# fugue-project/fugue

Measured on NVIDIA H100. Metric: transform() rows/sec, hash-partitioned (num=256) identity map, 8-col table, higher is better.
Workload: dtype int64+f64 (byte moves; u64 hash arithmetic)

## Files before the change

### fugue_b200/csrc/fb_partition.cu

```cuda
#include <stdlib.h>

#include <mutex>

#include "fb_common.cuh"

namespace {

constexpr int kBlock = 512;
constexpr int kItems = 8;
constexpr int kTile = kBlock * kItems;
constexpr int kWarps = kBlock / 32;
constexpr int kCtasPerSm = 2;

struct FbCols {
  const void* src[FB_MAX_COLS];
  void* dst[FB_MAX_COLS];
  int32_t width[FB_MAX_COLS];
  int32_t ncols;
};

struct ChunkGeom {
  int64_t nrows;
  int64_t full_rows;
  int64_t tiles_per_chunk;
// ... 278 lines not shown
  uint64_t* buf;
  uint32_t* delta;
  uint32_t* cursor;
  uint32_t* bin_start;
  uint32_t* cnt;
  uint32_t* scanw;
  uint16_t* pid_sorted;
  uint32_t nbp;
};

template <typename T, bool kFull>
__device__ __forceinline__ void load_col(const void* __restrict__ src, int64_t warp_row0, int warp_rows,
                                         unsigned lane, T (&v)[kItems]) {
  const T* __restrict__ p = (const T*)src + warp_row0 + lane;
#pragma unroll
  for (int r = 0; r < kItems; ++r)
    if (kFull || r * 32 + (int)lane < warp_rows) v[r] = __ldg(p + r * 32);
}

template <typename T, bool kFull>
__device__ __forceinline__ void move_columns(const FbCols& cols, const TileCtx& cx,
                                             const uint32_t (&pos)[kItems], const uint32_t (&dst)[kItems],
                                             int64_t warp_row0, int warp_rows, int tile_rows,
                                             unsigned lane, int& phase) {
  int c = 0;
  while (c < cols.ncols && cols.width[c] != (int)sizeof(T)) ++c;
  if (c >= cols.ncols) return;
  T v[kItems];
  load_col<T, kFull>(cols.src[c], warp_row0, warp_rows, lane, v);
  while (c < cols.ncols) {
    T* __restrict__ buf = (T*)(cx.buf + (size_t)(phase & 1) * kTile);
#pragma unroll
    for (int r = 0; r < kItems; ++r) buf[pos[r]] = v[r];
    int nxt = c + 1;
    while (nxt < cols.ncols && cols.width[nxt] != (int)sizeof(T)) ++nxt;
    if (nxt < cols.ncols) load_col<T, kFull>(cols.src[nxt], warp_row0, warp_rows, lane, v);
    __syncthreads();
    T* __restrict__ out = (T*)cols.dst[c];
#pragma unroll
    for (int k = 0; k < kItems; ++k) {
      const int j = k * kBlock + (int)threadIdx.x;
      if (kFull || j < tile_rows) out[dst[k]] = buf[j];
    }
    ++phase;
    c = nxt;
  }
}

template <bool kSingleU64, int kBits, bool kFull, bool kAll8>
__device__ __forceinline__ void scatter_tile(const FbKeys& keys, const FbDiv& dv, const uint32_t num,
                                             const FbCols& cols, const TileCtx& cx,
                                             const int64_t tile_row0, const int tile_rows, int& phase) {
  const unsigned lane = threadIdx.x & 31, warp = threadIdx.x >> 5;
  const unsigned lt = fb_lanemask_lt();
  const uint32_t nb = num + 1;
  const uint32_t nbp = cx.nbp;
  uint32_t* __restrict__ my_cnt = cx.cnt + warp * nbp;
  const int64_t warp_row0 = tile_row0 + (int64_t)warp * (32 * kItems);
  const int warp_rows = tile_rows - (int)warp * (32 * kItems);

  uint32_t pid[kItems];
#pragma unroll
  for (int r = 0; r < kItems; ++r) {
    const bool ok = kFull || (r * 32 + (int)lane) < warp_rows;
    pid[r] = ok ? compute_pid<kSingleU64>(keys, dv, warp_row0 + r * 32 + lane) : num;
  }

  uint32_t pos[kItems];
#pragma unroll
  for (int r = 0; r < kItems; ++r) {
    const unsigned m = match_lanes<kBits + (kFull ? 0 : 1)>(pid[r], 0xFFFFFFFFu);
    const unsigned before = __popc(m & lt);
    uint32_t old = 0;
    if (before == 0) {
      old = my_cnt[pid[r]];
      my_cnt[pid[r]] = old + __popc(m);
    }
    __syncwarp();
    old = __shfl_sync(0xFFFFFFFFu, old, __ffs(m) - 1);
    pos[r] = old + before;
  }
  __syncthreads();

  {
    const uint32_t per = (nb + kBlock - 1) / kBlock;
    const uint32_t b0 = threadIdx.x * per;
    uint32_t tot[kMaxPer];
    uint32_t sum = 0;
#pragma unroll
    for (int i = 0; i < kMaxPer; ++i) {
      tot[i] = 0;
      if ((uint32_t)i < per && b0 + i < nb) {
        uint32_t run = 0;
#pragma unroll
        for (int w = 0; w < kWarps; ++w) {
          const uint32_t t = cx.cnt[w * nbp + b0 + i];
          cx.cnt[w * nbp + b0 + i] = run;
          run += t;
        }
        tot[i] = run;
        sum += run;
      }
    }
    uint32_t x = sum;
#pragma unroll
    for (int o = 1; o < 32; o <<= 1) {
      const uint32_t y = __shfl_up_sync(0xFFFFFFFFu, x, o);
      if (lane >= (unsigned)o) x += y;
    }
    if (lane == 31) cx.scanw[warp] = x;
    __syncthreads();
    uint32_t run = x - sum;
    {
      const uint32_t wt = lane < kWarps ? cx.scanw[lane] : 0;
#pragma unroll
      for (int w = 0; w < kWarps; ++w) {
        const uint32_t v = __shfl_sync(0xFFFFFFFFu, wt, w);
        if ((unsigned)w < warp) run += v;
      }
    }
#pragma unroll
    for (int i = 0; i < kMaxPer; ++i) {
      if ((uint32_t)i < per && b0 + i < nb) {
        const uint32_t cur = cx.cursor[b0 + i];
        cx.bin_start[b0 + i] = run;
        cx.delta[b0 + i] = cur - run;
        cx.cursor[b0 + i] = cur + tot[i];
        run += tot[i];
      }
    }
  }
  __syncthreads();

#pragma unroll
  for (int r = 0; r < kItems; ++r) {
    pos[r] += cx.bin_start[pid[r]] + my_cnt[pid[r]];
    cx.pid_sorted[pos[r]] = (uint16_t)pid[r];
  }
  __syncthreads();
  uint32_t dst[kItems];
#pragma unroll
  for (int k = 0; k < kItems; ++k) {
    const int j = k * kBlock + (int)threadIdx.x;
    dst[k] = cx.delta[cx.pid_sorted[j]] + (uint32_t)j;
  }
  for (uint32_t i = threadIdx.x; i < (uint32_t)kWarps * nbp; i += kBlock) cx.cnt[i] = 0;

  move_columns<uint64_t, kFull>(cols, cx, pos, dst, warp_row0, warp_rows, tile_rows, lane, phase);
  if (!kAll8) {
    move_columns<uint32_t, kFull>(cols, cx, pos, dst, warp_row0, warp_rows, tile_rows, lane, phase);
    move_columns<uint16_t, kFull>(cols, cx, pos, dst, warp_row0, warp_rows, tile_rows, lane, phase);
    move_columns<uint8_t, kFull>(cols, cx, pos, dst, warp_row0, warp_rows, tile_rows, lane, phase);
  }
  __syncthreads();
}

template <bool kSingleU64, int kBits, bool kAll8>
__global__ void __launch_bounds__(kBlock, kCtasPerSm)
fb_scatter_kernel(FbKeys keys, FbDiv dv, uint32_t num, ChunkGeom g, int chunk0,
                  const uint32_t* __restrict__ chunk_base, const int64_t* __restrict__ part_offsets,
                  FbCols cols) {
  extern __shared__ __align__(128) uint64_t smem64[];
  TileCtx cx;
  cx.nbp = nb_padded(num);
  cx.buf = smem64;
  cx.delta = (uint32_t*)(smem64 + 2 * kTile);
  cx.cursor = cx.delta + cx.nbp;
  cx.bin_start = cx.cursor + cx.nbp;
  cx.cnt = cx.bin_start + cx.nbp;
  cx.scanw = cx.cnt + kWarps * cx.nbp;
  cx.pid_sorted = (uint16_t*)(cx.scanw + 32);

  const int chunk = chunk0 + (int)blockIdx.x;
  int64_t chunk_row0, chunk_row1;
  chunk_range(g, chunk, chunk_row0, chunk_row1);

  for (uint32_t b = threadIdx.x; b < cx.nbp; b += kBlock)
    cx.cursor[b] = b < num ? (uint32_t)part_offsets[b] + chunk_base[(size_t)chunk * num + b] : 0u;
  for (uint32_t i = threadIdx.x; i < (uint32_t)kWarps * cx.nbp; i += kBlock) cx.cnt[i] = 0;
  __syncthreads();

  int phase = 0;
  for (int64_t tile_row0 = chunk_row0; tile_row0 < chunk_row1; tile_row0 += kTile) {
    const int64_t left = chunk_row1 - tile_row0;
    if (left >= kTile)
      scatter_tile<kSingleU64, kBits, true, kAll8>(keys, dv, num, cols, cx, tile_row0, kTile, phase);
    else
      scatter_tile<kSingleU64, kBits, false, kAll8>(keys, dv, num, cols, cx, tile_row0, (int)left, phase);
  }
}

constexpr int kSwcMaxCols = 8;
constexpr uint32_t kSwcMaxNum = 256;

__device__ __forceinline__ uint32_t smem_u32(const void* p) { return (uint32_t)__cvta_generic_to_shared(p); }

__device__ __forceinline__ void mbar_init(uint32_t bar, uint32_t count) {
  asm volatile("mbarrier.init.shared::cta.b64 [%0], %1;" ::"r"(bar), "r"(count) : "memory");
}
__device__ __forceinline__ void mbar_expect_tx(uint32_t bar, uint32_t bytes) {
  asm volatile("mbarrier.arrive.expect_tx.shared::cta.b64 _, [%0], %1;" ::"r"(bar), "r"(bytes) : "memory");
}
__device__ __forceinline__ void mbar_arrive_relaxed(uint32_t bar) {
  asm volatile("mbarrier.arrive.relaxed.cta.shared::cta.b64 _, [%0];" ::"r"(bar) : "memory");
}
__device__ __forceinline__ void mbar_wait(uint32_t bar, uint32_t parity) {
  asm volatile(
      "{\n"
      ".reg .pred p;\n"
      "FB_WAIT:\n"
      "mbarrier.try_wait.parity.shared::cta.b64 p, [%0], %1;\n"
      "@p bra FB_DONE;\n"
      "bra FB_WAIT;\n"
      "FB_DONE:\n"
      "}\n" ::"r"(bar), "r"(parity)
      : "memory");
}
__device__ __forceinline__ uint64_t l2_policy_evict_first() {
  uint64_t pol;
  asm volatile("createpolicy.fractional.L2::evict_first.b64 %0, 1.0;" : "=l"(pol));
  return pol;
}
__device__ __forceinline__ uint64_t l2_policy_evict_last() {
  uint64_t pol;
  asm volatile("createpolicy.fractional.L2::evict_last.b64 %0, 1.0;" : "=l"(pol));
  return pol;
}
__device__ __forceinline__ void tma_load_1d(uint32_t dst_smem, const void* src, uint32_t bytes, uint32_t bar,
                                            uint64_t policy) {
  asm volatile(
      "cp.async.bulk.shared::cluster.global.mbarrier::complete_tx::bytes.L2::cache_hint [%0], [%1], %2, [%3], %4;"
      ::"r"(dst_smem), "l"(src), "r"(bytes), "r"(bar), "l"(policy)
      : "memory");
}

constexpr int kWsMoverWarps = 16, kWsRankWarps = 8;
constexpr int kWsMovers = kWsMoverWarps * 32, kWsRankers = kWsRankWarps * 32;
constexpr int kWsThreads = kWsMovers + kWsRankers + 128;
constexpr int kWsG = 4;
constexpr int kWsRankItems = 16;

struct WsUnits {
  const uint64_t* src[FB_MAX_COLS];
  uint64_t* dst[FB_MAX_COLS];
  int32_t nunits;
  int32_t per_group;
  int32_t ngroups;
};

struct WsMap {
  const uint64_t* src2[FB_MAX_COLS];
  uint64_t a[FB_MAX_COLS], b[FB_MAX_COLS], c[FB_MAX_COLS];
  int32_t mode[FB_MAX_COLS];
};

__device__ __forceinline__ uint64_t ws_apply_map(int mode, bool two, uint64_t x, uint64_t y, uint64_t a, uint64_t b,
                                                 uint64_t c) {
  if (mode == 1) {
    double r = __dmul_rn(__longlong_as_double((long long)a), __longlong_as_double((long long)x));
    if (two) r = __dadd_rn(r, __dmul_rn(__longlong_as_double((long long)b), __longlong_as_double((long long)y)));
    return (uint64_t)__double_as_longlong(__dadd_rn(r, __longlong_as_double((long long)c)));
  }
  if (mode == 2) return a * x + (two ? b * y : 0ULL) + c;
  return x;
}

template <int G, int RI>
__host__ __device__ inline size_t ws_book_bytes(uint32_t num, int ncols) {
  constexpr size_t kT = (size_t)kWsRankers * RI;
  const size_t nbp = nb_padded(num);
  const size_t E = (size_t)num * (G - 1);
  size_t b = 64 * 8;
  b += (size_t)ncols * E * 8;
  b += (kT + E) * 4;
  b += 6 * nbp * 4 + 64 * 4;
  b += ((E * 2 + 15) / 16) * 16;
  b += 2 * (size_t)kMetaBytes + 128;
  return b;
}

__device__ __forceinline__ void mbar_arrive(uint32_t bar) {
  asm volatile("mbarrier.arrive.shared::cta.b64 _, [%0];" ::"r"(bar) : "memory");
}
__device__ __forceinline__ void mover_sync() { asm volatile("bar.sync 1, %0;" ::"n"(kWsMovers) : "memory"); }
__device__ __forceinline__ void ranker_sync() { asm volatile("bar.sync 2, %0;" ::"n"(kWsRankers) : "memory"); }

template <int kBits, int G, int kWsRankItems, bool kMap>
__global__ void __launch_bounds__(kWsThreads, 1)
fb_scatter_ws_kernel(WsUnits units, uint32_t num, ChunkGeom g, int nstages,
                     const uint8_t* __restrict__ meta,
                     const uint32_t* __restrict__ chunk_base, const int64_t* __restrict__ part_offsets,
                     const __grid_constant__ WsMap map) {
  constexpr uint32_t T = (uint32_t)kWsRankers * kWsRankItems;
  static_assert(T == (uint32_t)kTile, "pass 1 ranks tiles of kTile rows");
  constexpr uint32_t GM = G - 1;
  constexpr uint32_t kStageBytes = T * 8;
  constexpr int kSlotRounds = ((int)T + (int)kSwcMaxNum * (G - 1) + kWsMovers - 1) / kWsMovers;
  constexpr int kEntryRoundsM = ((int)kSwcMaxNum * (G - 1) + kWsMovers - 1) / kWsMovers;
  constexpr int kEntryRoundsR = ((int)kSwcMaxNum * (G - 1) + kWsRankers - 1) / kWsRankers;
  extern __shared__ __align__(128) uint64_t smem64[];
  const uint32_t nbp = nb_padded(num);
  const uint32_t E = num * GM;
  const int grp = (int)blockIdx.x % units.ngroups;
  const int chunk_first = (int)blockIdx.x / units.ngroups, chunk_step = (int)gridDim.x / units.ngroups;
  const int u0 = grp * units.per_group;
  const int ncols = min(units.per_group, units.nunits - u0);
  uint64_t* ring = smem64;
  uint64_t* bars = ring + (size_t)nstages * T;
  uint64_t* carry = bars + 64;
  uint32_t* slotinfo = (uint32_t*)(carry + (size_t)ncols * E);
  uint32_t* wpos = slotinfo + T + E;
  uint32_t* kcnt = wpos + nbp;
  uint32_t* binfo = kcnt + nbp;
  uint32_t* bin_n = binfo + nbp;
  uint32_t* wstart = bin_n + nbp;
  uint32_t* wdelta = wstart + nbp;
  uint32_t* scanw = wdelta + nbp;
  uint16_t* carryinfo = (uint16_t*)(scanw + 64);
  uint8_t* metabuf = (uint8_t*)(((uintptr_t)(carryinfo + E) + 127) & ~(uintptr_t)127);

  const unsigned lane = threadIdx.x & 31, warp = threadIdx.x >> 5;
  const uint32_t bar_full = smem_u32(bars), bar_empty = smem_u32(bars + 16);
  const uint32_t bar_pid_full = smem_u32(bars + 32), bar_pid_empty = smem_u32(bars + 34);
  const uint32_t bar_slots_ready = smem_u32(bars + 36), bar_slots_free = smem_u32(bars + 37);
  const uint32_t bar_flush_done = smem_u32(bars + 38);
  const uint32_t bar_carry_read = smem_u32(bars + 40);

  if (threadIdx.x == 0) {
    for (int s = 0; s < nstages; ++s) {
      mbar_init(bar_full + 8 * s, 1);
      mbar_init(bar_empty + 8 * s, kWsMoverWarps);
    }
    for (int i = 0; i < 2; ++i) {
      mbar_init(bar_pid_full + 8 * i, 1);
      mbar_init(bar_pid_empty + 8 * i, kWsRankWarps);
    }
    mbar_init(bar_slots_ready, kWsRankWarps);
    mbar_init(bar_slots_free, kWsMoverWarps);
    mbar_init(bar_flush_done, kWsMoverWarps);
    mbar_init(bar_carry_read, kWsMoverWarps);
    mbar_init(bar_carry_read + 8, kWsMoverWarps);
    asm volatile("fence.mbarrier_init.release.cluster;" ::: "memory");
  }
  __syncthreads();

  if (warp >= kWsMoverWarps + kWsRankWarps) {
    if (warp == kWsMoverWarps + kWsRankWarps && lane == 0) {
      const uint64_t pol = l2_policy_evict_first(), meta_pol = l2_policy_evict_last();
      const uint32_t ring_s = smem_u32(ring), meta_s = smem_u32(metabuf);
      uint32_t s = 0, ph = 0, seq = 0;
      int chunk = chunk_first;
      int64_t r0 = 0, r1 = 0, t0 = 0;
      bool have = chunk < g.nchunks_full;
      if (have) { chunk_range(g, chunk, r0, r1); t0 = r0; }
      auto load_pid = [&](int64_t row0, uint32_t q) {
        const uint32_t b = q & 1, pp = (q >> 1) & 1;
        mbar_wait(bar_pid_empty + 8 * b, pp ^ 1);
        mbar_expect_tx(bar_pid_full + 8 * b, kMetaBytes);
        tma_load_1d(meta_s + b * kMetaBytes, meta + (size_t)(row0 / T) * kMetaBytes, kMetaBytes,
                    bar_pid_full + 8 * b, meta_pol);
      };
      if (have) load_pid(t0, 0);
      while (have) {
        int nchunk = chunk;
        int64_t nr0 = r0, nr1 = r1, nt0 = t0 + T;
        bool nhave = true;
        if (nt0 >= r1) {
          nchunk = chunk + chunk_step;
          nhave = nchunk < g.nchunks_full;
          if (nhave) { chunk_range(g, nchunk, nr0, nr1); nt0 = nr0; }
        }
        if (nhave) load_pid(nt0, seq + 1);
        for (int u = u0; u < u0 + ncols; ++u) {
          mbar_wait(bar_empty + 8 * s, ph ^ 1);
          mbar_expect_tx(bar_full + 8 * s, kStageBytes);
          tma_load_1d(ring_s + s * kStageBytes, units.src[u] + t0, kStageBytes, bar_full + 8 * s, pol);
          if (++s == (uint32_t)nstages) { s = 0; ph ^= 1; }
          if constexpr (kMap) {
            if (map.src2[u] != nullptr) {
              mbar_wait(bar_empty + 8 * s, ph ^ 1);
              mbar_expect_tx(bar_full + 8 * s, kStageBytes);
              tma_load_1d(ring_s + s * kStageBytes, map.src2[u] + t0, kStageBytes, bar_full + 8 * s, pol);
              if (++s == (uint32_t)nstages) { s = 0; ph ^= 1; }
            }
          }
        }
        chunk = nchunk; r0 = nr0; r1 = nr1; t0 = nt0; have = nhave;
        ++seq;
      }
    }
    return;
  }

  if (warp >= kWsMoverWarps) {
    const unsigned rw = warp - kWsMoverWarps;
    const unsigned rtid = threadIdx.x - kWsMovers;
    uint32_t seq = 0, cseq = 0;
    for (int chunk = chunk_first; chunk < g.nchunks_full; chunk += chunk_step, ++cseq) {
      int64_t r0, r1;
      chunk_range(g, chunk, r0, r1);
      if (cseq > 0) mbar_wait(bar_flush_done, (cseq - 1) & 1);
      ranker_sync();
      for (uint32_t b = rtid; b < nbp; b += kWsRankers) {
        const uint32_t p0 = b < num ? (uint32_t)part_offsets[b] + chunk_base[(size_t)chunk * num + b] : 0u;
        wpos[b] = p0 & ~GM;
        kcnt[b] = (p0 & GM) | ((p0 & GM) << 8);
      }
      ranker_sync();
      for (int64_t t0 = r0; t0 < r1; t0 += T, ++seq) {
        const uint32_t pb = seq & 1, pph = (seq >> 1) & 1;
        mbar_wait(bar_pid_full + 8 * pb, pph);
        const uint8_t* __restrict__ rec = metabuf + pb * kMetaBytes;
        uint32_t pr[kWsRankItems];
#pragma unroll
        for (int r = 0; r < kWsRankItems; ++r) {
          const uint32_t row = r * kWsRankers + rtid;
          pr[r] = ((uint32_t)rec[row] << 16) | ((const uint16_t*)(rec + kMetaRank))[row];
        }
        const uint32_t b = rtid;
        uint32_t n = 0, w = 0, kold = 0, phold = 0, wp_old = 0;
        if (b < num) n = ((const uint16_t*)(rec + kMetaCnt))[b];
        __syncwarp();
        if (lane == 0) mbar_arrive_relaxed(bar_pid_empty + 8 * pb);
        if (b < num) {
          const uint32_t kc = kcnt[b];
          kold = kc & 0xFFu;
          phold = kc >> 8;
          wp_old = wpos[b];
          const uint32_t end = wp_old + kold + n;
          const uint32_t aend = end & ~GM;
          if (aend > wp_old) {
            w = aend - wp_old;
            wpos[b] = aend;
            kcnt[b] = end - aend;
          } else {
            kcnt[b] = (kold + n) | (phold << 8);
          }
          binfo[b] = kold | (phold << 4) | (w << 8);
          bin_n[b] = n;
        }
        uint32_t xw = w;
#pragma unroll
        for (int o = 1; o < 32; o <<= 1) {
          const uint32_t yw = __shfl_up_sync(0xFFFFFFFFu, xw, o);
          if (lane >= (unsigned)o) xw += yw;
        }
        if (lane == 31) scanw[8 + rw] = xw;
        ranker_sync();
        uint32_t bw = xw - w;
        {
          const uint32_t tw = lane < kWsRankWarps ? scanw[8 + lane] : 0;
#pragma unroll
          for (int wi = 0; wi < kWsRankWarps; ++wi) {
            const uint32_t vw = __shfl_sync(0xFFFFFFFFu, tw, wi);
            if ((unsigned)wi < rw) bw += vw;
          }
        }
        if (seq > 0) mbar_wait(bar_slots_free, (seq - 1) & 1);
        if (b < num) {
          wstart[b] = bw;
          wdelta[b] = wp_old - bw;
        }
        if (rtid == kWsRankers - 1) scanw[40] = bw + w;
        ranker_sync();
#pragma unroll
        for (int r = 0; r < kWsRankItems; ++r) {
          const uint32_t pb2 = pr[r] >> 16;
          const uint32_t bi = binfo[pb2];
          const uint32_t i = (bi & 0xFu) + (pr[r] & 0xFFFFu);
          const uint32_t ww = bi >> 8;
          const uint32_t row = r * kWsRankers + rtid;
          if (i < ww) slotinfo[wstart[pb2] + i] = (pb2 << 16) | row;
          else carryinfo[pb2 * GM + (i - ww)] = (uint16_t)row;
        }
#pragma unroll
        for (int q = 0; q < kEntryRoundsR; ++q) {
          const uint32_t e = q * kWsRankers + rtid;
          if (e < E) {
            const uint32_t eb = e / GM, i = e - eb * GM;
            const uint32_t bi = binfo[eb];
            const uint32_t ko = bi & 0xFu, po = (bi >> 4) & 0xFu, ww = bi >> 8;
            const uint32_t nn = bin_n[eb];
            const uint32_t desc = i < po ? 0xFFFFu : T + e;
            if (i < ko) {
              if (i < ww) slotinfo[wstart[eb] + i] = (eb << 16) | desc;
              else carryinfo[e] = (uint16_t)desc;
            }
            if (ww + i >= ko + nn) carryinfo[e] = 0xFFFFu;
          }
        }
        ranker_sync();
        if (lane == 0) mbar_arrive(bar_slots_ready);
      }
    }
    return;
  }

  uint32_t s = 0, ph = 0, seq = 0, astep = 0, wstep = 0;
  for (int chunk = chunk_first; chunk < g.nchunks_full; chunk += chunk_step) {
    int64_t r0, r1;
    chunk_range(g, chunk, r0, r1);
    for (int64_t t0 = r0; t0 < r1; t0 += T, ++seq) {
      mbar_wait(bar_slots_ready, seq & 1);
      const uint32_t W = scanw[40];
      uint32_t srcd[kSlotRounds], dst[kSlotRounds];
#pragma unroll
      for (int k = 0; k < kSlotRounds; ++k) {
        const uint32_t j = k * kWsMovers + threadIdx.x;
        srcd[k] = 0xFFFFu;
        dst[k] = 0;
        if (j < W) {
          const uint32_t info = slotinfo[j];
          srcd[k] = info & 0xFFFFu;
          dst[k] = wdelta[info >> 16] + j;
        }
      }
      uint32_t csrc[kEntryRoundsM];
#pragma unroll
      for (int q = 0; q < kEntryRoundsM; ++q) {
        const uint32_t e = q * kWsMovers + threadIdx.x;
        csrc[q] = e < E ? (uint32_t)carryinfo[e] : 0xFFFFu;
      }
      __syncwarp();
      if (lane == 0) mbar_arrive(bar_slots_free);

      uint64_t cv_prev[kEntryRoundsM];
      for (int u = 0; u < ncols; ++u) {
        mbar_wait(bar_full + 8 * s, ph);
        const uint64_t* __restrict__ st = ring + (size_t)s * T;
        uint64_t* __restrict__ out = units.dst[u0 + u];
        const uint64_t* __restrict__ cbuf = carry + (size_t)u * E;
        uint64_t v[kSlotRounds], cv[kEntryRoundsM];
        uint32_t s2 = s;
        bool two = false;
        if constexpr (kMap) {
          const int mode = map.mode[u0 + u];
          two = map.src2[u0 + u] != nullptr;
          const uint64_t* __restrict__ st2 = st;
          if (two) {
            s2 = s + 1 == (uint32_t)nstages ? 0 : s + 1;
            mbar_wait(bar_full + 8 * s2, s2 == 0 ? ph ^ 1 : ph);
            st2 = ring + (size_t)s2 * T;
          }
          const uint64_t ma = map.a[u0 + u], mb = map.b[u0 + u], mc = map.c[u0 + u];
#pragma unroll
          for (int k = 0; k < kSlotRounds; ++k)
            if (srcd[k] != 0xFFFFu)
              v[k] = srcd[k] < T ? ws_apply_map(mode, two, st[srcd[k]], st2[srcd[k]], ma, mb, mc) : cbuf[srcd[k] - T];
#pragma unroll
          for (int q = 0; q < kEntryRoundsM; ++q)
            if (csrc[q] != 0xFFFFu)
              cv[q] = csrc[q] < T ? ws_apply_map(mode, two, st[csrc[q]], st2[csrc[q]], ma, mb, mc) : cbuf[csrc[q] - T];
        } else {
#pragma unroll
          for (int k = 0; k < kSlotRounds; ++k)
            if (srcd[k] != 0xFFFFu) v[k] = srcd[k] < T ? st[srcd[k]] : cbuf[srcd[k] - T];
#pragma unroll
          for (int q = 0; q < kEntryRoundsM; ++q)
            if (csrc[q] != 0xFFFFu) cv[q] = csrc[q] < T ? st[csrc[q]] : cbuf[csrc[q] - T];
        }
#pragma unroll
        for (int k = 0; k < kSlotRounds; ++k)
          if (srcd[k] != 0xFFFFu) out[dst[k]] = v[k];
        __syncwarp();
        if (lane == 0) {
          mbar_arrive_relaxed(bar_empty + 8 * s);
          if (kMap && two) mbar_arrive_relaxed(bar_empty + 8 * s2);
          mbar_arrive_relaxed(bar_carry_read + 8 * (astep & 1));
        }
        ++astep;
        if (++s == (uint32_t)nstages) { s = 0; ph ^= 1; }
        if (kMap && two) {
          if (++s == (uint32_t)nstages) { s = 0; ph ^= 1; }
        }
        if (u > 0) {
          mbar_wait(bar_carry_read + 8 * (wstep & 1), (wstep >> 1) & 1);
          ++wstep;
          uint64_t* __restrict__ pbuf = carry + (size_t)(u - 1) * E;
#pragma unroll
          for (int q = 0; q < kEntryRoundsM; ++q) {
            const uint32_t e = q * kWsMovers + threadIdx.x;
            if (csrc[q] != 0xFFFFu) pbuf[e] = cv_prev[q];
          }
        }
#pragma unroll
        for (int q = 0; q < kEntryRoundsM; ++q) cv_prev[q] = cv[q];
      }
      {
        mbar_wait(bar_carry_read + 8 * (wstep & 1), (wstep >> 1) & 1);
        ++wstep;
        uint64_t* __restrict__ pbuf = carry + (size_t)(ncols - 1) * E;
#pragma unroll
        for (int q = 0; q < kEntryRoundsM; ++q) {
          const uint32_t e = q * kWsMovers + threadIdx.x;
          if (csrc[q] != 0xFFFFu) pbuf[e] = cv_prev[q];
        }
      }
    }
    mover_sync();
    for (int u = 0; u < ncols; ++u) {
      uint64_t* __restrict__ out = units.dst[u0 + u];
      const uint64_t* __restrict__ cbuf = carry + (size_t)u * E;
#pragma unroll
      for (int q = 0; q < kEntryRoundsM; ++q) {
        const uint32_t e = q * kWsMovers + threadIdx.x;
        if (e < E) {
          const uint32_t b = e / GM, i = e - b * GM;
          const uint32_t kc = kcnt[b];
          if (i < (kc & 0xFFu) && i >= (kc >> 8)) out[wpos[b] + i] = cbuf[e];
        }
      }
    }
    __syncwarp();
    if (lane == 0) mbar_arrive(bar_flush_done);
  }
}

__global__ void fb_bits_to_bytes_kernel(const uint8_t* __restrict__ bits, int64_t bit_offset,
                                        int64_t nrows, uint8_t* __restrict__ out) {
  int64_t i = (int64_t)blockIdx.x * blockDim.x + threadIdx.x;
  int64_t stride = (int64_t)gridDim.x * blockDim.x;
  for (; i < nrows; i += stride) {
    int64_t j = i + bit_offset;
    out[i] = (bits[j >> 3] >> (j & 7)) & 1;
  }
}

__global__ void fb_bytes_to_bits_kernel(const uint8_t* __restrict__ bytes, int64_t nrows,
                                        uint8_t* __restrict__ out, unsigned long long* null_count) {
  int64_t nbytes = (nrows + 7) >> 3;
  int64_t i = (int64_t)blockIdx.x * blockDim.x + threadIdx.x;
  int64_t stride = (int64_t)gridDim.x * blockDim.x;
  unsigned long long nulls = 0;
  for (; i < nbytes; i += stride) {
    uint8_t v = 0;
#pragma unroll
    for (int k = 0; k < 8; ++k) {
      int64_t r = i * 8 + k;
      if (r < nrows) {
        if (bytes[r]) v |= (uint8_t)(1u << k);
        else ++nulls;
      }
    }
    out[i] = v;
  }
  if (null_count != nullptr && nulls) atomicAdd(null_count, nulls);
}

inline int bits_for(uint32_t num) { return num <= 16 ? 4 : (num <= 256 ? 8 : 10); }

#define FB_DISPATCH_SB(single, bits, LAUNCH)                 \
  do {                                                       \
    if (single) {                                            \
      if (bits == 4) LAUNCH(true, 4);                        \
      else if (bits == 8) LAUNCH(true, 8);                   \
      else LAUNCH(true, 10);                                 \
    } else {                                                 \
      if (bits == 4) LAUNCH(false, 4);                       \
      else if (bits == 8) LAUNCH(false, 8);                  \
      else LAUNCH(false, 10);                                \
    }                                                        \
  } while (0)

template <typename K>
cudaError_t optin(K kernel, size_t bytes) {
  return cudaFuncSetAttribute(kernel, cudaFuncAttributeMaxDynamicSharedMemorySize, (int)bytes);
}

cudaError_t ensure_smem_optin(int dev) {
  static std::mutex mu;
  static uint64_t done = 0;
  std::lock_guard<std::mutex> lock(mu);
  if (dev >= 0 && dev < 64 && (done >> dev) & 1) return cudaSuccess;
  const size_t sc = scatter_smem_bytes(FB_MAX_PARTITIONS);
  const size_t hs = (size_t)kHistWarps * FB_MAX_PARTITIONS * sizeof(uint32_t);
  cudaError_t e = cudaSuccess;
#define FB_OPTIN(S, B)                                                   \
  do {                                                                   \
    if (e == cudaSuccess) e = optin(fb_scatter_kernel<S, B, true>, sc);  \
    if (e == cudaSuccess) e = optin(fb_scatter_kernel<S, B, false>, sc); \
    if (e == cudaSuccess) e = optin(fb_hist_kernel<S, B>, hs);           \
  } while (0)
  {
    int smem_max = 0;
    if (e == cudaSuccess) e = cudaDeviceGetAttribute(&smem_max, cudaDevAttrMaxSharedMemoryPerBlockOptin, dev);
    if (e == cudaSuccess) e = optin(fb_scatter_ws_kernel<4, kWsG, kWsRankItems, false>, (size_t)smem_max);
    if (e == cudaSuccess) e = optin(fb_scatter_ws_kernel<8, kWsG, kWsRankItems, false>, (size_t)smem_max);
    if (e == cudaSuccess) e = optin(fb_scatter_ws_kernel<4, kWsG, kWsRankItems, true>, (size_t)smem_max);
    if (e == cudaSuccess) e = optin(fb_scatter_ws_kernel<8, kWsG, kWsRankItems, true>, (size_t)smem_max);
  }
  if (e == cudaSuccess) e = optin(fb_rank_kernel<true, 4, true>, kRankStageBytes);
  if (e == cudaSuccess) e = optin(fb_rank_kernel<true, 8, true>, kRankStageBytes);
  if (e == cudaSuccess) e = optin(fb_rank_kernel<false, 4, true>, kRankStageBytes);
  if (e == cudaSuccess) e = optin(fb_rank_kernel<false, 8, true>, kRankStageBytes);
  FB_OPTIN(true, 4); FB_OPTIN(true, 8); FB_OPTIN(true, 10);
  FB_OPTIN(false, 4); FB_OPTIN(false, 8); FB_OPTIN(false, 10);
#undef FB_OPTIN
  if (e == cudaSuccess && dev >= 0 && dev < 64) done |= (1ull << dev);
  return e;
}

bool single_u64_key(int nkeys, const int32_t* widths, const uint8_t* const* valid) {
  return nkeys == 1 && widths[0] == 8 && (valid == nullptr || valid[0] == nullptr);
}

int fill_keys(FbKeys& k, int nkeys, const void* const* ptrs, const int32_t* widths,
              const uint8_t* const* valid) {
  FB_CHECK(nkeys >= 1 && nkeys <= FB_MAX_KEYS, "nkeys=%d out of range [1,%d]", nkeys, FB_MAX_KEYS);
  memset(&k, 0, sizeof(k));
  k.nkeys = nkeys;
  k.digit_shift = -1;
  for (int i = 0; i < nkeys; ++i) {
    FB_CHECK(widths[i] == 1 || widths[i] == 2 || widths[i] == 4 || widths[i] == 8,
             "key %d has unsupported width %d", i, widths[i]);
    FB_CHECK(ptrs[i] != nullptr, "key %d pointer is NULL", i);
    k.ptr[i] = ptrs[i];
    k.width[i] = widths[i];
    k.valid[i] = valid ? valid[i] : nullptr;
  }
  return 0;
}

struct PlanLayout {
  size_t hist_bytes;
  size_t pid_offset;
  size_t total_bytes;
};

PlanLayout plan_layout(const ChunkGeom& g, uint32_t num) {
  PlanLayout l;
  l.hist_bytes = (((size_t)g.nchunks * num * sizeof(uint32_t)) + 255) & ~(size_t)255;
  l.pid_offset = l.hist_bytes + 256;
  l.total_bytes = l.pid_offset + (num <= kSwcMaxNum ? (size_t)(g.full_rows / kTile) * kMetaBytes : 0) + 256;
  return l;
}

}

extern "C" {

size_t fb_partition_scratch_bytes(int dev, int64_t nrows, uint32_t num_partitions) {
  if (nrows < 0 || num_partitions == 0) return 0;
  ChunkGeom g = make_geom(dev, nrows);
  return plan_layout(g, num_partitions).total_bytes;
}

int fb_partition_ids(int dev, void* stream, int64_t nrows, int nkeys, const void* const* key_ptrs,
                     const int32_t* key_widths, const uint8_t* const* key_valid,
                     uint32_t num_partitions, uint32_t* out_pids) {
  FB_CHECK(nrows >= 0, "nrows < 0");
  FB_CHECK(num_partitions >= 1, "num_partitions must be >= 1");
  if (nrows == 0) return 0;
  FbDeviceGuard guard(dev);
  FB_CHECK(guard.ok, "cannot select device %d", dev);
  FbKeys k;
  if (int rc = fill_keys(k, nkeys, key_ptrs, key_widths, key_valid)) return rc;
  FbDiv dv = fb_make_div(num_partitions);
  int64_t blocks = (nrows + 255) / 256;
  int64_t maxb = (int64_t)fb_sm_count(dev) * 16;
  if (blocks > maxb) blocks = maxb;
  cudaStream_t st = (cudaStream_t)stream;
  if (single_u64_key(nkeys, key_widths, key_valid))
    fb_pid_kernel<true><<<(unsigned)blocks, 256, 0, st>>>(k, dv, nrows, out_pids);
  else
    fb_pid_kernel<false><<<(unsigned)blocks, 256, 0, st>>>(k, dv, nrows, out_pids);
  FB_CUDA(cudaGetLastError());
  return 0;
}

int fb_row_hash64(int dev, void* stream, int64_t nrows, int nkeys, const void* const* key_ptrs,
                  const int32_t* key_widths, const uint8_t* const* key_valid, uint64_t* out_hash) {
  FB_CHECK(nrows >= 0, "nrows < 0");
  if (nrows == 0) return 0;
  FbDeviceGuard guard(dev);
  FB_CHECK(guard.ok, "cannot select device %d", dev);
  FbKeys k;
  if (int rc = fill_keys(k, nkeys, key_ptrs, key_widths, key_valid)) return rc;
  int64_t blocks = (nrows + 255) / 256;
  int64_t maxb = (int64_t)fb_sm_count(dev) * 16;
  if (blocks > maxb) blocks = maxb;
  fb_row_hash_kernel<<<(unsigned)blocks, 256, 0, (cudaStream_t)stream>>>(k, nrows, out_hash);
  FB_CUDA(cudaGetLastError());
  return 0;
}

static int plan_impl(int dev, void* stream, int64_t nrows, const FbKeys& k, bool single,
                     uint32_t num_partitions, void* scratch, size_t scratch_bytes,
                     int64_t* out_part_offsets) {
  FB_CHECK(nrows >= 0, "nrows < 0");
  FB_CHECK(nrows < ((int64_t)1 << 32), "nrows=%lld exceeds the 2^32-1 rows one call handles",
           (long long)nrows);
  FB_CHECK(num_partitions >= 1 && num_partitions <= FB_MAX_PARTITIONS,
           "num_partitions=%u out of range [1,%d]", num_partitions, FB_MAX_PARTITIONS);
  FB_CHECK(out_part_offsets != nullptr, "out_part_offsets is NULL");
  FbDeviceGuard guard(dev);
  FB_CHECK(guard.ok, "cannot select device %d", dev);
  cudaStream_t st = (cudaStream_t)stream;
  if (nrows == 0) {
    FB_CUDA(cudaMemsetAsync(out_part_offsets, 0, sizeof(int64_t) * ((size_t)num_partitions + 1), st));
    return 0;
  }
  ChunkGeom g = make_geom(dev, nrows);
  PlanLayout l = plan_layout(g, num_partitions);
  FB_CHECK(scratch != nullptr && scratch_bytes >= l.total_bytes,
           "scratch too small: need %zu bytes, got %zu", l.total_bytes, scratch_bytes);
  FbDiv dv = fb_make_div(num_partitions);
  uint32_t* hist = (uint32_t*)scratch;
  size_t smem = (size_t)kHistWarps * num_partitions * sizeof(uint32_t);
  FB_CUDA(ensure_smem_optin(dev));
  const int bits = bits_for(num_partitions);
  int hist_chunk0 = 0;
  if (num_partitions <= kSwcMaxNum && g.nchunks_full > 0) {
    uint8_t* meta = (uint8_t*)scratch + l.pid_offset;
#define FB_LAUNCH_RANK(S, B, STAGED)                                                                  \
  fb_rank_kernel<S, B, STAGED><<<g.nchunks_full, kRankBlock, STAGED ? kRankStageBytes : 0, st>>>( \
      k, dv, num_partitions, g, hist, meta)
    if (single) {
      if (bits == 4) FB_LAUNCH_RANK(true, 4, true);
      else FB_LAUNCH_RANK(true, 8, true);
    } else if (k.digit_shift >= 0) {
      if (bits == 4) FB_LAUNCH_RANK(false, 4, true);
      else FB_LAUNCH_RANK(false, 8, true);
    } else {
      if (bits == 4) FB_LAUNCH_RANK(false, 4, false);
      else FB_LAUNCH_RANK(false, 8, false);
    }
#undef FB_LAUNCH_RANK
    FB_CUDA(cudaGetLastError());
    hist_chunk0 = g.nchunks_full;
  }
  if (hist_chunk0 < g.nchunks) {
#define FB_LAUNCH_HIST(S, B)                                                                       \
  fb_hist_kernel<S, B><<<g.nchunks - hist_chunk0, kHistBlock, smem, st>>>(k, dv, num_partitions, g, \
                                                                          hist_chunk0, hist)
    FB_DISPATCH_SB(single, bits, FB_LAUNCH_HIST);
#undef FB_LAUNCH_HIST
    FB_CUDA(cudaGetLastError());
  }
  fb_scan_chunks_kernel<<<num_partitions, 256, 0, st>>>(hist, num_partitions, g.nchunks, out_part_offsets);
  FB_CUDA(cudaGetLastError());
  fb_scan_parts_kernel<<<1, 1024, 0, st>>>(out_part_offsets, num_partitions);
  FB_CUDA(cudaGetLastError());
  return 0;
}

int fb_partition_plan(int dev, void* stream, int64_t nrows, int nkeys, const void* const* key_ptrs,
                      const int32_t* key_widths, const uint8_t* const* key_valid,
                      uint32_t num_partitions, void* scratch, size_t scratch_bytes,
                      int64_t* out_part_offsets) {
  FbKeys k;
  if (nrows == 0) {
    memset(&k, 0, sizeof(k));
    k.nkeys = 1;
    k.digit_shift = -1;
    return plan_impl(dev, stream, 0, k, false, num_partitions, scratch, scratch_bytes, out_part_offsets);
  }
  if (int rc = fill_keys(k, nkeys, key_ptrs, key_widths, key_valid)) return rc;
  return plan_impl(dev, stream, nrows, k, single_u64_key(nkeys, key_widths, key_valid), num_partitions,
                   scratch, scratch_bytes, out_part_offsets);
}

__global__ void fb_map_tail_kernel(int ncols, const void* const* __restrict__ x_ptrs, const fb_map_unit* __restrict__ maps,
                                   int64_t row0, int64_t nrows, uint64_t* __restrict__ tmp) {
  const int64_t n = nrows - row0;
  for (int64_t i = (int64_t)blockIdx.x * blockDim.x + threadIdx.x; i < n * ncols; i += (int64_t)gridDim.x * blockDim.x) {
    const int c = (int)(i / n);
    const int64_t r = row0 + i % n;
    const fb_map_unit m = maps[c];
    const uint64_t x = ((const uint64_t*)x_ptrs[c])[r];
    const uint64_t y = m.src2 != nullptr ? ((const uint64_t*)m.src2)[r] : 0;
    tmp[(size_t)c * kTile + (size_t)(i % n)] = ws_apply_map(m.mode, m.src2 != nullptr, x, y, m.a, m.b, m.c);
  }
}

static int apply_impl(int dev, void* stream, int64_t nrows, const FbKeys& k, bool single,
                      uint32_t num_partitions, const void* scratch, size_t scratch_bytes,
                      const int64_t* part_offsets, int ncols, const void* const* col_ptrs,
                      const int32_t* col_widths, void* const* out_col_ptrs, int sm_reserve = 0,
                      const fb_map_unit* maps = nullptr, void* tail_tmp = nullptr, int cols_per_launch_req = 0) {
  FB_CHECK(nrows >= 0 && nrows < ((int64_t)1 << 32), "nrows out of range");
  FB_CHECK(num_partitions >= 1 && num_partitions <= FB_MAX_PARTITIONS,
           "num_partitions=%u out of range [1,%d]", num_partitions, FB_MAX_PARTITIONS);
  FB_CHECK(ncols >= 0, "ncols < 0");
  if (nrows == 0 || ncols == 0) return 0;
  FbDeviceGuard guard(dev);
  FB_CHECK(guard.ok, "cannot select device %d", dev);
  ChunkGeom g = make_geom(dev, nrows);
  PlanLayout l = plan_layout(g, num_partitions);
  FB_CHECK(scratch != nullptr && scratch_bytes >= l.total_bytes, "scratch too small");
  FbDiv dv = fb_make_div(num_partitions);
  cudaStream_t st = (cudaStream_t)stream;
  const size_t smem = scatter_smem_bytes(num_partitions);
  FB_CUDA(ensure_smem_optin(dev));
  const int bits = bits_for(num_partitions);

  for (int c = 0; c < ncols; ++c) {
    const int w = col_widths[c];
    FB_CHECK(w == 1 || w == 2 || w == 4 || w == 8, "column %d has unsupported width %d", c, w);
    FB_CHECK(col_ptrs[c] != nullptr && out_col_ptrs[c] != nullptr, "column %d pointer is NULL", c);
  }

  const void* const* gen_src = col_ptrs;
  auto launch_generic = [&](const int* idx, int n, int chunk0, int nch) -> int {
    for (int c0 = 0; c0 < n && nch > 0; c0 += FB_MAX_COLS) {
      FbCols cols;
      memset(&cols, 0, sizeof(cols));
      cols.ncols = n - c0 < FB_MAX_COLS ? n - c0 : FB_MAX_COLS;
      bool all8 = true;
      for (int c = 0; c < cols.ncols; ++c) {
        cols.src[c] = gen_src[idx[c0 + c]];
        cols.dst[c] = out_col_ptrs[idx[c0 + c]];
        cols.width[c] = col_widths[idx[c0 + c]];
        all8 = all8 && cols.width[c] == 8;
      }
#define FB_LAUNCH_SCATTER(S, B)                                                                        \
  do {                                                                                                 \
    if (all8)                                                                                          \
// ... 230 lines not shown
```

Measured before the change: 16.10 billion.

## Assign each CTA a contiguous run of chunks to drop per-chunk flush barriers

The warp-specialized scatter kernel now gives each CTA one contiguous range of tiles instead of striding over chunks. Ranker state is seeded once from the first chunk's base, and the producer, ranker and mover loops iterate over tiles directly. This removes the per-chunk carry flush and the flush_done barrier between chunks, so the pipeline no longer drains at chunk boundaries. It relies on consecutive chunks' write positions continuing seamlessly. It also shifts load balance to the per-run split, which may be uneven when chunks do not divide evenly across runs.

```diff
diff --git a/fugue_b200/csrc/fb_partition.cu b/fugue_b200/csrc/fb_partition.cu
--- a/fugue_b200/csrc/fb_partition.cu
+++ b/fugue_b200/csrc/fb_partition.cu
@@ -604,7 +604,12 @@
   const uint32_t nbp = nb_padded(num);
   const uint32_t E = num * GM;
   const int grp = (int)blockIdx.x % units.ngroups;
-  const int chunk_first = (int)blockIdx.x / units.ngroups, chunk_step = (int)gridDim.x / units.ngroups;
+  const uint32_t run = blockIdx.x / (uint32_t)units.ngroups, nruns = gridDim.x / (uint32_t)units.ngroups;
+  const uint32_t c_lo = run * (uint32_t)g.nchunks_full / nruns;
+  const uint32_t c_hi = (run + 1) * (uint32_t)g.nchunks_full / nruns;
+  const uint32_t tile_lo = c_lo * (uint32_t)g.tiles_per_chunk;
+  const uint32_t tile_hi = min(c_hi * (uint32_t)g.tiles_per_chunk, (uint32_t)(g.full_rows / kTile));
+  const uint32_t run_tiles = tile_hi - tile_lo;
   const int u0 = grp * units.per_group;
   const int ncols = min(units.per_group, units.nunits - u0);
   uint64_t* ring = smem64;
@@ -625,7 +630,6 @@
   const uint32_t bar_full = smem_u32(bars), bar_empty = smem_u32(bars + 16);
   const uint32_t bar_pid_full = smem_u32(bars + 32), bar_pid_empty = smem_u32(bars + 34);
   const uint32_t bar_slots_ready = smem_u32(bars + 36), bar_slots_free = smem_u32(bars + 37);
-  const uint32_t bar_flush_done = smem_u32(bars + 38);
   const uint32_t bar_carry_read = smem_u32(bars + 40);
 
   if (threadIdx.x == 0) {
@@ -639,7 +643,6 @@
     }
     mbar_init(bar_slots_ready, kWsRankWarps);
     mbar_init(bar_slots_free, kWsMoverWarps);
-    mbar_init(bar_flush_done, kWsMoverWarps);
     mbar_init(bar_carry_read, kWsMoverWarps);
     mbar_init(bar_carry_read + 8, kWsMoverWarps);
     asm volatile("fence.mbarrier_init.release.cluster;" ::: "memory");
@@ -651,28 +654,17 @@
       const uint64_t pol = l2_policy_evict_first(), meta_pol = l2_policy_evict_last();
       const uint32_t ring_s = smem_u32(ring), meta_s = smem_u32(metabuf);
       uint32_t s = 0, ph = 0, seq = 0;
-      int chunk = chunk_first;
-      int64_t r0 = 0, r1 = 0, t0 = 0;
-      bool have = chunk < g.nchunks_full;
-      if (have) { chunk_range(g, chunk, r0, r1); t0 = r0; }
-      auto load_pid = [&](int64_t row0, uint32_t q) {
+      auto load_pid = [&](uint32_t tile, uint32_t q) {
         const uint32_t b = q & 1, pp = (q >> 1) & 1;
         mbar_wait(bar_pid_empty + 8 * b, pp ^ 1);
         mbar_expect_tx(bar_pid_full + 8 * b, kMetaBytes);
-        tma_load_1d(meta_s + b * kMetaBytes, meta + (size_t)(row0 / T) * kMetaBytes, kMetaBytes,
+        tma_load_1d(meta_s + b * kMetaBytes, meta + (size_t)tile * kMetaBytes, kMetaBytes,
                     bar_pid_full + 8 * b, meta_pol);
       };
-      if (have) load_pid(t0, 0);
-      while (have) {
-        int nchunk = chunk;
-        int64_t nr0 = r0, nr1 = r1, nt0 = t0 + T;
-        bool nhave = true;
-        if (nt0 >= r1) {
-          nchunk = chunk + chunk_step;
-          nhave = nchunk < g.nchunks_full;
-          if (nhave) { chunk_range(g, nchunk, nr0, nr1); nt0 = nr0; }
-        }
-        if (nhave) load_pid(nt0, seq + 1);
+      load_pid(tile_lo, 0);
+      for (uint32_t tile = tile_lo; tile < tile_hi; ++tile, ++seq) {
+        if (tile + 1 < tile_hi) load_pid(tile + 1, seq + 1);
+        const size_t t0 = (size_t)tile * T;
         for (int u = u0; u < u0 + ncols; ++u) {
           mbar_wait(bar_empty + 8 * s, ph ^ 1);
           mbar_expect_tx(bar_full + 8 * s, kStageBytes);
@@ -687,8 +679,6 @@
             }
           }
         }
-        chunk = nchunk; r0 = nr0; r1 = nr1; t0 = nt0; have = nhave;
-        ++seq;
       }
     }
     return;
@@ -697,224 +687,212 @@
   if (warp >= kWsMoverWarps) {
     const unsigned rw = warp - kWsMoverWarps;
     const unsigned rtid = threadIdx.x - kWsMovers;
-    uint32_t seq = 0, cseq = 0;
-    for (int chunk = chunk_first; chunk < g.nchunks_full; chunk += chunk_step, ++cseq) {
-      int64_t r0, r1;
-      chunk_range(g, chunk, r0, r1);
-      if (cseq > 0) mbar_wait(bar_flush_done, (cseq - 1) & 1);
+    uint32_t seq = 0;
+    for (uint32_t b = rtid; b < nbp; b += kWsRankers) {
+      const uint32_t p0 = b < num ? (uint32_t)part_offsets[b] + chunk_base[(size_t)c_lo * num + b] : 0u;
+      wpos[b] = p0 & ~GM;
+      kcnt[b] = (p0 & GM) | ((p0 & GM) << 8);
+    }
+    ranker_sync();
+    for (; seq < run_tiles; ++seq) {
+      const uint32_t pb = seq & 1, pph = (seq >> 1) & 1;
+      mbar_wait(bar_pid_full + 8 * pb, pph);
+      const uint8_t* __restrict__ rec = metabuf + pb * kMetaBytes;
+      uint32_t pr[kWsRankItems];
+#pragma unroll
+      for (int r = 0; r < kWsRankItems; ++r) {
+        const uint32_t row = r * kWsRankers + rtid;
+        pr[r] = ((uint32_t)rec[row] << 16) | ((const uint16_t*)(rec + kMetaRank))[row];
+      }
+      const uint32_t b = rtid;
+      uint32_t n = 0, w = 0, kold = 0, phold = 0, wp_old = 0;
+      if (b < num) n = ((const uint16_t*)(rec + kMetaCnt))[b];
+      __syncwarp();
+      if (lane == 0) mbar_arrive_relaxed(bar_pid_empty + 8 * pb);
+      if (b < num) {
+        const uint32_t kc = kcnt[b];
+        kold = kc & 0xFFu;
+        phold = kc >> 8;
+        wp_old = wpos[b];
+        const uint32_t end = wp_old + kold + n;
+        const uint32_t aend = end & ~GM;
+        if (aend > wp_old) {
+          w = aend - wp_old;
+          wpos[b] = aend;
+          kcnt[b] = end - aend;
+        } else {
+          kcnt[b] = (kold + n) | (phold << 8);
+        }
+        binfo[b] = kold | (phold << 4) | (w << 8);
+        bin_n[b] = n;
+      }
+      uint32_t xw = w;
+#pragma unroll
+      for (int o = 1; o < 32; o <<= 1) {
+        const uint32_t yw = __shfl_up_sync(0xFFFFFFFFu, xw, o);
+        if (lane >= (unsigned)o) xw += yw;
+      }
+      if (lane == 31) scanw[8 + rw] = xw;
       ranker_sync();
-      for (uint32_t b = rtid; b < nbp; b += kWsRankers) {
-        const uint32_t p0 = b < num ? (uint32_t)part_offsets[b] + chunk_base[(size_t)chunk * num + b] : 0u;
-        wpos[b] = p0 & ~GM;
-        kcnt[b] = (p0 & GM) | ((p0 & GM) << 8);
-      }
+      uint32_t bw = xw - w;
+      {
+        const uint32_t tw = lane < kWsRankWarps ? scanw[8 + lane] : 0;
+#pragma unroll
+        for (int wi = 0; wi < kWsRankWarps; ++wi) {
+          const uint32_t vw = __shfl_sync(0xFFFFFFFFu, tw, wi);
+          if ((unsigned)wi < rw) bw += vw;
+        }
+      }
+      if (seq > 0) mbar_wait(bar_slots_free, (seq - 1) & 1);
+      if (b < num) {
+        wstart[b] = bw;
+        wdelta[b] = wp_old - bw;
+      }
+      if (rtid == kWsRankers - 1) scanw[40] = bw + w;
       ranker_sync();
-      for (int64_t t0 = r0; t0 < r1; t0 += T, ++seq) {
-        const uint32_t pb = seq & 1, pph = (seq >> 1) & 1;
-        mbar_wait(bar_pid_full + 8 * pb, pph);
-        const uint8_t* __restrict__ rec = metabuf + pb * kMetaBytes;
-        uint32_t pr[kWsRankItems];
-#pragma unroll
-        for (int r = 0; r < kWsRankItems; ++r) {
-          const uint32_t row = r * kWsRankers + rtid;
-          pr[r] = ((uint32_t)rec[row] << 16) | ((const uint16_t*)(rec + kMetaRank))[row];
+#pragma unroll
+      for (int r = 0; r < kWsRankItems; ++r) {
+        const uint32_t pb2 = pr[r] >> 16;
+        const uint32_t bi = binfo[pb2];
+        const uint32_t i = (bi & 0xFu) + (pr[r] & 0xFFFFu);
+        const uint32_t ww = bi >> 8;
+        const uint32_t row = r * kWsRankers + rtid;
+        if (i < ww) slotinfo[wstart[pb2] + i] = (pb2 << 16) | row;
+        else carryinfo[pb2 * GM + (i - ww)] = (uint16_t)row;
+      }
+#pragma unroll
+      for (int q = 0; q < kEntryRoundsR; ++q) {
+        const uint32_t e = q * kWsRankers + rtid;
+        if (e < E) {
+          const uint32_t eb = e / GM, i = e - eb * GM;
+          const uint32_t bi = binfo[eb];
+          const uint32_t ko = bi & 0xFu, po = (bi >> 4) & 0xFu, ww = bi >> 8;
+          const uint32_t nn = bin_n[eb];
+          const uint32_t desc = i < po ? 0xFFFFu : T + e;
+          if (i < ko) {
+            if (i < ww) slotinfo[wstart[eb] + i] = (eb << 16) | desc;
+            else carryinfo[e] = (uint16_t)desc;
+          }
+          if (ww + i >= ko + nn) carryinfo[e] = 0xFFFFu;
         }
-        const uint32_t b = rtid;
-        uint32_t n = 0, w = 0, kold = 0, phold = 0, wp_old = 0;
-        if (b < num) n = ((const uint16_t*)(rec + kMetaCnt))[b];
-        __syncwarp();
-        if (lane == 0) mbar_arrive_relaxed(bar_pid_empty + 8 * pb);
-        if (b < num) {
-          const uint32_t kc = kcnt[b];
-          kold = kc & 0xFFu;
-          phold = kc >> 8;
-          wp_old = wpos[b];
-          const uint32_t end = wp_old + kold + n;
-          const uint32_t aend = end & ~GM;
-          if (aend > wp_old) {
-            w = aend - wp_old;
-            wpos[b] = aend;
-            kcnt[b] = end - aend;
-          } else {
-            kcnt[b] = (kold + n) | (phold << 8);
-          }
-          binfo[b] = kold | (phold << 4) | (w << 8);
-          bin_n[b] = n;
+      }
+      ranker_sync();
+      if (lane == 0) mbar_arrive(bar_slots_ready);
+    }
+    return;
+  }
+
+  uint32_t s = 0, ph = 0, seq = 0, astep = 0, wstep = 0;
+  for (; seq < run_tiles; ++seq) {
+    mbar_wait(bar_slots_ready, seq & 1);
+    const uint32_t W = scanw[40];
+    uint32_t srcd[kSlotRounds], dst[kSlotRounds];
+#pragma unroll
+    for (int k = 0; k < kSlotRounds; ++k) {
+      const uint32_t j = k * kWsMovers + threadIdx.x;
+      srcd[k] = 0xFFFFu;
+      dst[k] = 0;
+      if (j < W) {
+        const uint32_t info = slotinfo[j];
+        srcd[k] = info & 0xFFFFu;
+        dst[k] = wdelta[info >> 16] + j;
+      }
+    }
+    uint32_t csrc[kEntryRoundsM];
+#pragma unroll
+    for (int q = 0; q < kEntryRoundsM; ++q) {
+      const uint32_t e = q * kWsMovers + threadIdx.x;
+      csrc[q] = e < E ? (uint32_t)carryinfo[e] : 0xFFFFu;
+    }
+    __syncwarp();
+    if (lane == 0) mbar_arrive(bar_slots_free);
+
+    uint64_t cv_prev[kEntryRoundsM];
+    for (int u = 0; u < ncols; ++u) {
+      mbar_wait(bar_full + 8 * s, ph);
+      const uint64_t* __restrict__ st = ring + (size_t)s * T;
+      uint64_t* __restrict__ out = units.dst[u0 + u];
+      const uint64_t* __restrict__ cbuf = carry + (size_t)u * E;
+      uint64_t v[kSlotRounds], cv[kEntryRoundsM];
+      uint32_t s2 = s;
+      bool two = false;
+      if constexpr (kMap) {
+        const int mode = map.mode[u0 + u];
+        two = map.src2[u0 + u] != nullptr;
+        const uint64_t* __restrict__ st2 = st;
+        if (two) {
+          s2 = s + 1 == (uint32_t)nstages ? 0 : s + 1;
+          mbar_wait(bar_full + 8 * s2, s2 == 0 ? ph ^ 1 : ph);
+          st2 = ring + (size_t)s2 * T;
         }
-        uint32_t xw = w;
-#pragma unroll
-        for (int o = 1; o < 32; o <<= 1) {
-          const uint32_t yw = __shfl_up_sync(0xFFFFFFFFu, xw, o);
-          if (lane >= (unsigned)o) xw += yw;
-        }
-        if (lane == 31) scanw[8 + rw] = xw;
-        ranker_sync();
-        uint32_t bw = xw - w;
-        {
-          const uint32_t tw = lane < kWsRankWarps ? scanw[8 + lane] : 0;
-#pragma unroll
-          for (int wi = 0; wi < kWsRankWarps; ++wi) {
-            const uint32_t vw = __shfl_sync(0xFFFFFFFFu, tw, wi);
-            if ((unsigned)wi < rw) bw += vw;
-          }
-        }
-        if (seq > 0) mbar_wait(bar_slots_free, (seq - 1) & 1);
-        if (b < num) {
-          wstart[b] = bw;
-          wdelta[b] = wp_old - bw;
-        }
-        if (rtid == kWsRankers - 1) scanw[40] = bw + w;
-        ranker_sync();
-#pragma unroll
-        for (int r = 0; r < kWsRankItems; ++r) {
-          const uint32_t pb2 = pr[r] >> 16;
-          const uint32_t bi = binfo[pb2];
-          const uint32_t i = (bi & 0xFu) + (pr[r] & 0xFFFFu);
-          const uint32_t ww = bi >> 8;
-          const uint32_t row = r * kWsRankers + rtid;
-          if (i < ww) slotinfo[wstart[pb2] + i] = (pb2 << 16) | row;
-          else carryinfo[pb2 * GM + (i - ww)] = (uint16_t)row;
-        }
-#pragma unroll
-        for (int q = 0; q < kEntryRoundsR; ++q) {
-          const uint32_t e = q * kWsRankers + rtid;
-          if (e < E) {
-            const uint32_t eb = e / GM, i = e - eb * GM;
-            const uint32_t bi = binfo[eb];
-            const uint32_t ko = bi & 0xFu, po = (bi >> 4) & 0xFu, ww = bi >> 8;
-            const uint32_t nn = bin_n[eb];
-            const uint32_t desc = i < po ? 0xFFFFu : T + e;
-            if (i < ko) {
-              if (i < ww) slotinfo[wstart[eb] + i] = (eb << 16) | desc;
-              else carryinfo[e] = (uint16_t)desc;
-            }
-            if (ww + i >= ko + nn) carryinfo[e] = 0xFFFFu;
-          }
-        }
-        ranker_sync();
-        if (lane == 0) mbar_arrive(bar_slots_ready);
-      }
-    }
-    return;
-  }
-
-  uint32_t s = 0, ph = 0, seq = 0, astep = 0, wstep = 0;
-  for (int chunk = chunk_first; chunk < g.nchunks_full; chunk += chunk_step) {
-    int64_t r0, r1;
-    chunk_range(g, chunk, r0, r1);
-    for (int64_t t0 = r0; t0 < r1; t0 += T, ++seq) {
-      mbar_wait(bar_slots_ready, seq & 1);
-      const uint32_t W = scanw[40];
-      uint32_t srcd[kSlotRounds], dst[kSlotRounds];
-#pragma unroll
-      for (int k = 0; k < kSlotRounds; ++k) {
-        const uint32_t j = k * kWsMovers + threadIdx.x;
-        srcd[k] = 0xFFFFu;
-        dst[k] = 0;
-        if (j < W) {
-          const uint32_t info = slotinfo[j];
-          srcd[k] = info & 0xFFFFu;
-          dst[k] = wdelta[info >> 16] + j;
-        }
-      }
-      uint32_t csrc[kEntryRoundsM];
-#pragma unroll
-      for (int q = 0; q < kEntryRoundsM; ++q) {
-        const uint32_t e = q * kWsMovers + threadIdx.x;
-        csrc[q] = e < E ? (uint32_t)carryinfo[e] : 0xFFFFu;
-      }
+        const uint64_t ma = map.a[u0 + u], mb = map.b[u0 + u], mc = map.c[u0 + u];
+#pragma unroll
+        for (int k = 0; k < kSlotRounds; ++k)
+          if (srcd[k] != 0xFFFFu)
+            v[k] = srcd[k] < T ? ws_apply_map(mode, two, st[srcd[k]], st2[srcd[k]], ma, mb, mc) : cbuf[srcd[k] - T];
+#pragma unroll
+        for (int q = 0; q < kEntryRoundsM; ++q)
+          if (csrc[q] != 0xFFFFu)
+            cv[q] = csrc[q] < T ? ws_apply_map(mode, two, st[csrc[q]], st2[csrc[q]], ma, mb, mc) : cbuf[csrc[q] - T];
+      } else {
+#pragma unroll
+        for (int k = 0; k < kSlotRounds; ++k)
+          if (srcd[k] != 0xFFFFu) v[k] = srcd[k] < T ? st[srcd[k]] : cbuf[srcd[k] - T];
+#pragma unroll
+        for (int q = 0; q < kEntryRoundsM; ++q)
+          if (csrc[q] != 0xFFFFu) cv[q] = csrc[q] < T ? st[csrc[q]] : cbuf[csrc[q] - T];
+      }
+#pragma unroll
+      for (int k = 0; k < kSlotRounds; ++k)
+        if (srcd[k] != 0xFFFFu) out[dst[k]] = v[k];
       __syncwarp();
-      if (lane == 0) mbar_arrive(bar_slots_free);
-
-      uint64_t cv_prev[kEntryRoundsM];
-      for (int u = 0; u < ncols; ++u) {
-        mbar_wait(bar_full + 8 * s, ph);
-        const uint64_t* __restrict__ st = ring + (size_t)s * T;
-        uint64_t* __restrict__ out = units.dst[u0 + u];
-        const uint64_t* __restrict__ cbuf = carry + (size_t)u * E;
-        uint64_t v[kSlotRounds], cv[kEntryRoundsM];
-        uint32_t s2 = s;
-        bool two = false;
-        if constexpr (kMap) {
-          const int mode = map.mode[u0 + u];
-          two = map.src2[u0 + u] != nullptr;
-          const uint64_t* __restrict__ st2 = st;
-          if (two) {
-            s2 = s + 1 == (uint32_t)nstages ? 0 : s + 1;
-            mbar_wait(bar_full + 8 * s2, s2 == 0 ? ph ^ 1 : ph);
-            st2 = ring + (size_t)s2 * T;
-          }
-          const uint64_t ma = map.a[u0 + u], mb = map.b[u0 + u], mc = map.c[u0 + u];
-#pragma unroll
-          for (int k = 0; k < kSlotRounds; ++k)
-            if (srcd[k] != 0xFFFFu)
-              v[k] = srcd[k] < T ? ws_apply_map(mode, two, st[srcd[k]], st2[srcd[k]], ma, mb, mc) : cbuf[srcd[k] - T];
-#pragma unroll
-          for (int q = 0; q < kEntryRoundsM; ++q)
-            if (csrc[q] != 0xFFFFu)
-              cv[q] = csrc[q] < T ? ws_apply_map(mode, two, st[csrc[q]], st2[csrc[q]], ma, mb, mc) : cbuf[csrc[q] - T];
-        } else {
-#pragma unroll
-          for (int k = 0; k < kSlotRounds; ++k)
-            if (srcd[k] != 0xFFFFu) v[k] = srcd[k] < T ? st[srcd[k]] : cbuf[srcd[k] - T];
-#pragma unroll
-          for (int q = 0; q < kEntryRoundsM; ++q)
-            if (csrc[q] != 0xFFFFu) cv[q] = csrc[q] < T ? st[csrc[q]] : cbuf[csrc[q] - T];
-        }
-#pragma unroll
-        for (int k = 0; k < kSlotRounds; ++k)
-          if (srcd[k] != 0xFFFFu) out[dst[k]] = v[k];
-        __syncwarp();
-        if (lane == 0) {
-          mbar_arrive_relaxed(bar_empty + 8 * s);
-          if (kMap && two) mbar_arrive_relaxed(bar_empty + 8 * s2);
-          mbar_arrive_relaxed(bar_carry_read + 8 * (astep & 1));
-        }
-        ++astep;
+      if (lane == 0) {
+        mbar_arrive_relaxed(bar_empty + 8 * s);
+        if (kMap && two) mbar_arrive_relaxed(bar_empty + 8 * s2);
+        mbar_arrive_relaxed(bar_carry_read + 8 * (astep & 1));
+      }
+      ++astep;
+      if (++s == (uint32_t)nstages) { s = 0; ph ^= 1; }
+      if (kMap && two) {
         if (++s == (uint32_t)nstages) { s = 0; ph ^= 1; }
-        if (kMap && two) {
-          if (++s == (uint32_t)nstages) { s = 0; ph ^= 1; }
-        }
-        if (u > 0) {
-          mbar_wait(bar_carry_read + 8 * (wstep & 1), (wstep >> 1) & 1);
-          ++wstep;
-          uint64_t* __restrict__ pbuf = carry + (size_t)(u - 1) * E;
-#pragma unroll
-          for (int q = 0; q < kEntryRoundsM; ++q) {
-            const uint32_t e = q * kWsMovers + threadIdx.x;
-            if (csrc[q] != 0xFFFFu) pbuf[e] = cv_prev[q];
-          }
-        }
-#pragma unroll
-        for (int q = 0; q < kEntryRoundsM; ++q) cv_prev[q] = cv[q];
-      }
-      {
+      }
+      if (u > 0) {
         mbar_wait(bar_carry_read + 8 * (wstep & 1), (wstep >> 1) & 1);
         ++wstep;
-        uint64_t* __restrict__ pbuf = carry + (size_t)(ncols - 1) * E;
+        uint64_t* __restrict__ pbuf = carry + (size_t)(u - 1) * E;
 #pragma unroll
         for (int q = 0; q < kEntryRoundsM; ++q) {
           const uint32_t e = q * kWsMovers + threadIdx.x;
           if (csrc[q] != 0xFFFFu) pbuf[e] = cv_prev[q];
         }
       }
-    }
-    mover_sync();
-    for (int u = 0; u < ncols; ++u) {
-      uint64_t* __restrict__ out = units.dst[u0 + u];
-      const uint64_t* __restrict__ cbuf = carry + (size_t)u * E;
+#pragma unroll
+      for (int q = 0; q < kEntryRoundsM; ++q) cv_prev[q] = cv[q];
+    }
+    {
+      mbar_wait(bar_carry_read + 8 * (wstep & 1), (wstep >> 1) & 1);
+      ++wstep;
+      uint64_t* __restrict__ pbuf = carry + (size_t)(ncols - 1) * E;
 #pragma unroll
       for (int q = 0; q < kEntryRoundsM; ++q) {
         const uint32_t e = q * kWsMovers + threadIdx.x;
-        if (e < E) {
-          const uint32_t b = e / GM, i = e - b * GM;
-          const uint32_t kc = kcnt[b];
-          if (i < (kc & 0xFFu) && i >= (kc >> 8)) out[wpos[b] + i] = cbuf[e];
-        }
-      }
-    }
-    __syncwarp();
-    if (lane == 0) mbar_arrive(bar_flush_done);
+        if (csrc[q] != 0xFFFFu) pbuf[e] = cv_prev[q];
+      }
+    }
+  }
+  mover_sync();
+  for (int u = 0; u < ncols; ++u) {
+    uint64_t* __restrict__ out = units.dst[u0 + u];
+    const uint64_t* __restrict__ cbuf = carry + (size_t)u * E;
+#pragma unroll
+    for (int q = 0; q < kEntryRoundsM; ++q) {
+      const uint32_t e = q * kWsMovers + threadIdx.x;
+      if (e < E) {
+        const uint32_t b = e / GM, i = e - b * GM;
+        const uint32_t kc = kcnt[b];
+        if (i < (kc & 0xFFu) && i >= (kc >> 8)) out[wpos[b] + i] = cbuf[e];
+      }
+    }
   }
 }
 
```

Measured after the change: 16.27 billion, median of 6. 1.1% higher.
